# ghostop14/gr-clenabled

Measured on AMD Instinct MI355X. Metric: MSamples/sec (complex-float) through clFFT 4096 fwd + window + shift, higher is better.
Workload: dtype f32; 1 GPU; BASELINE configs[1]: forward clFFT 4096-pt complex, blackman window + fftshift, 16384 frames/step/GPU device-resident (1 GiB in+out); fft_size=4096, parallelism=replica-per-gpu x1

## Files before the change

gr-clenabled_amd/csrc/fft.hip:

```cpp
#include <cmath>
#include <cstdlib>
#include <vector>

#include "common.h"
#include "fft_core.hpp"
#include "fft_mr.h"

using namespace fftc;
#ifndef MI355_FFT_WPE
#define MI355_FFT_WPE 3
#endif

namespace {

typedef float f2v __attribute__((ext_vector_type(2)));

template <int N, bool REAL, class G>
__device__ __forceinline__ void load_group(c32 (&v)[16], const void *__restrict__ in, int grp, int tid, int nframes, int in_xor)
{
    using P = Plan<N>;
    constexpr int TH = G::TH, PTS = G::PTS, F = G::F, R0 = P::radix(0), B0 = N / R0;
    const int frames_left = nframes - grp * F;
    if constexpr (N <= 64) {
        (void)in_xor;
#pragma unroll
        for (int k = 0; k < 16; k++) {
            const unsigned e = (unsigned)(tid + TH * k);
            const bool ok = (int)(e / N) < frames_left;
            if constexpr (REAL) {
                const float x = __builtin_nontemporal_load((const float *)in + (size_t)grp * PTS + (ok ? e : 0u));
                v[k] = mk(ok ? x : 0.f, 0.f);
            } else {
                const f2v x = __builtin_nontemporal_load((const f2v *)in + (size_t)grp * PTS + (ok ? e : 0u));
                v[k] = ok ? mk(x.x, x.y) : mk(0.f, 0.f);
            }
        }
        return;
    }
#pragma unroll
    for (int q = 0; q < 16 / R0; q++) {
        const int g = tid + TH * q, fr = g / B0;
        const bool ok = (F == 1) || fr < frames_left;
        const unsigned off = (unsigned)((ok ? fr * N : 0) + (g % B0));
#pragma unroll
        for (int r = 0; r < R0; r++) {
            const unsigned e = off + (unsigned)((r * B0) ^ in_xor);
            if constexpr (REAL) {
                const float x = __builtin_nontemporal_load((const float *)in + (size_t)grp * PTS + e);
                v[q * R0 + r] = mk(ok ? x : 0.f, 0.f);
            } else {
                const f2v x = __builtin_nontemporal_load((const f2v *)in + (size_t)grp * PTS + e);
                v[q * R0 + r] = ok ? mk(x.x, x.y) : mk(0.f, 0.f);
            }
        }
    }
}

template <int N, int SIGN, bool REAL, int PF, class G>
__global__ __launch_bounds__(G::TH, (N <= 4096 ? (PF == 2 ? 2 : MI355_FFT_WPE) : 1)) void k_fft(const void *__restrict__ in, c32 *__restrict__ out,
                                                                 const float *__restrict__ window,
                                                                 const c32 *__restrict__ twtab, int nframes, int ngroups,
                                                                 int shift)
{
    using P = Plan<N>;
    constexpr int TH = G::TH, PTS = G::PTS, F = G::F, NP = P::NP;
    constexpr bool SMALL = N <= 64;
    constexpr int PAD = (N / P::radix(0)) > 1 ? (N / P::radix(0)) : 1;
    constexpr int LDS_SLOTS = SMALL ? PTS + (PTS / N) * PAD : (NP > 1 ? PTS : 1);
    __shared__ c32 lds[LDS_SLOTS];
    const int tid0 = threadIdx.x;
    const int in_xor = (SIGN > 0 && shift) ? (N >> 1) : 0;
    const int out_xor = (SIGN < 0 && shift) ? (N >> 1) : 0;

    TwRegs<N> tw;
    load_twiddles<N, false, G>(tw, tid0, twtab);
    constexpr int R0 = P::radix(0), B0 = N / R0;
    float win[16];
    if constexpr (SMALL) {
        win[0] = window[tid0 % N];
    } else {
#pragma unroll
        for (int q = 0; q < 16 / R0; q++) {
            const int j = (tid0 + TH * q) % B0;
#pragma unroll
            for (int r = 0; r < R0; r++) win[q * R0 + r] = window[j + ((r * B0) ^ in_xor)];
        }
    }

    auto body = [&](c32 (&cur)[16], int grp, int tid) {
        const int frames_left = nframes - grp * F;
        c32 v[16];
        if constexpr (SMALL) {
            const float wv = win[0];
            const int pos = (tid % N) ^ in_xor, fr0 = tid / N;
#pragma unroll
            for (int k = 0; k < 16; k++) {
                const int fr = fr0 + k * (TH / N);
                lds[fr * (N + PAD) + pos] = scale(cur[k], wv);
            }
            __syncthreads();
#pragma unroll
            for (int q = 0; q < 16 / R0; q++) {
                const int g = tid + TH * q, base = (g / B0) * (N + PAD) + (g % B0);
#pragma unroll
                for (int r = 0; r < R0; r++) v[q * R0 + r] = lds[base + r * B0];
            }
            __syncthreads();
        } else {
#pragma unroll
            for (int s = 0; s < 16; s++) v[s] = scale(cur[s], win[s]);
        }
        transform_regs<N, SIGN, false, G>(v, tw, lds, tid);
        if constexpr (SMALL) {
            constexpr int RL = P::radix(NP - 1), BL = N / RL;
            if constexpr (NP > 1) __syncthreads();
#pragma unroll
            for (int q = 0; q < 16 / RL; q++) {
                const int g = tid + TH * q, base = (g / BL) * (N + PAD) + (g % BL);
#pragma unroll
                for (int s = 0; s < RL; s++) lds[base + ((orev<RL>(s) * BL) ^ out_xor)] = v[q * RL + s];
            }
            __syncthreads();
            f2v *__restrict__ out_g = (f2v *)out + (size_t)grp * PTS;
            const int pos = tid % N, fr0 = tid / N;
#pragma unroll
            for (int k = 0; k < 16; k++) {
                const int fr = fr0 + k * (TH / N);
                if (fr < frames_left) {
                    const c32 z = lds[fr * (N + PAD) + pos];
                    f2v o;
                    o.x = z.x;
                    o.y = z.y;
                    __builtin_nontemporal_store(o, out_g + tid + TH * k);
                }
            }
        } else {
            constexpr int RL = P::radix(NP - 1), BL = N / RL;
            f2v *__restrict__ out_g = (f2v *)out + (size_t)grp * PTS;
#pragma unroll
            for (int q = 0; q < 16 / RL; q++) {
                const int g = tid + TH * q, fr = g / BL;
                const unsigned off = (unsigned)(fr * N + (g % BL));
                if ((F == 1) || fr < frames_left) {
#pragma unroll
                    for (int s = 0; s < RL; s++) {
                        f2v o;
                        o.x = v[q * RL + s].x;
                        o.y = v[q * RL + s].y;
                        __builtin_nontemporal_store(o, out_g + off + (unsigned)((orev<RL>(s) * BL) ^ out_xor));
                    }
                }
            }
        }
        if constexpr (NP > 1 || SMALL) __syncthreads();
    };
    const int stride = gridDim.x;
    if constexpr (PF == 2) {
        c32 b0[16], b1[16], b2[16];
        int grp = blockIdx.x;
        if (grp < ngroups) load_group<N, REAL, G>(b0, in, grp, tid0, nframes, in_xor);
        if (grp + stride < ngroups) load_group<N, REAL, G>(b1, in, grp + stride, tid0, nframes, in_xor);
#define MI355_FFT_STEP(CUR, FREE)                                                                   \
        {                                                                                           \
            if (grp >= ngroups) break;                                                              \
            int tid = tid0;                                                                         \
            asm volatile("" : "+v"(tid));                                                           \
            if (grp + 2 * stride < ngroups) load_group<N, REAL, G>(FREE, in, grp + 2 * stride, tid, nframes, in_xor); \
            __builtin_amdgcn_sched_barrier(0);                                                      \
            body(CUR, grp, tid);                                                                    \
            grp += stride;                                                                          \
        }
        for (;;) {
            MI355_FFT_STEP(b0, b2)
            MI355_FFT_STEP(b1, b0)
            MI355_FFT_STEP(b2, b1)
        }
#undef MI355_FFT_STEP
    } else {
        c32 cur[16];
        if ((int)blockIdx.x < ngroups) load_group<N, REAL, G>(cur, in, blockIdx.x, tid0, nframes, in_xor);
        for (int grp = blockIdx.x; grp < ngroups; grp += stride) {
            int tid = tid0;
            asm volatile("" : "+v"(tid));
            c32 nxt[16];
            if constexpr (PF == 1) {
                const int gnext = grp + stride;
                if (gnext < ngroups) load_group<N, REAL, G>(nxt, in, gnext, tid, nframes, in_xor);
                __builtin_amdgcn_sched_barrier(0);
            } else if (grp != (int)blockIdx.x) {
                load_group<N, REAL, G>(cur, in, grp, tid, nframes, in_xor);
            }
            body(cur, grp, tid);
            if constexpr (PF == 1) {
#pragma unroll
                for (int s = 0; s < 16; s++) cur[s] = nxt[s];
            }
        }
    }
}

typedef float f4v __attribute__((ext_vector_type(4)));
__host__ __device__ constexpr float cos128(int m)
{
    constexpr float t[128] = {1.0f, 0.99879545f, 0.99518472f, 0.989176512f, 0.980785251f, 0.970031261f, 0.956940353f, 0.941544056f, 0.923879504f, 0.903989315f, 0.881921291f, 0.857728601f, 0.831469595f, 0.803207517f, 0.773010433f, 0.740951121f, 0.707106769f, 0.671558976f, 0.634393275f, 0.59569931f, 0.555570245f, 0.514102757f, 0.471396744f, 0.427555084f, 0.382683426f, 0.336889863f, 0.290284663f, 0.242980182f, 0.195090324f, 0.146730468f, 0.0980171412f, 0.0490676761f, 0.0f, -0.0490676761f, -0.0980171412f, -0.146730468f, -0.195090324f, -0.242980182f, -0.290284663f, -0.336889863f, -0.382683426f, -0.427555084f, -0.471396744f, -0.514102757f, -0.555570245f, -0.59569931f, -0.634393275f, -0.671558976f, -0.707106769f, -0.740951121f, -0.773010433f, -0.803207517f, -0.831469595f, -0.857728601f, -0.881921291f, -0.903989315f, -0.923879504f, -0.941544056f, -0.956940353f, -0.970031261f, -0.980785251f, -0.989176512f, -0.99518472f, -0.99879545f, -1.0f, -0.99879545f, -0.99518472f, -0.989176512f, -0.980785251f, -0.970031261f, -0.956940353f, -0.941544056f, -0.923879504f, -0.903989315f, -0.881921291f, -0.857728601f, -0.831469595f, -0.803207517f, -0.773010433f, -0.740951121f, -0.707106769f, -0.671558976f, -0.634393275f, -0.59569931f, -0.555570245f, -0.514102757f, -0.471396744f, -0.427555084f, -0.382683426f, -0.336889863f, -0.290284663f, -0.242980182f, -0.195090324f, -0.146730468f, -0.0980171412f, -0.0490676761f, 0.0f, 0.0490676761f, 0.0980171412f, 0.146730468f, 0.195090324f, 0.242980182f, 0.290284663f, 0.336889863f, 0.382683426f, 0.427555084f, 0.471396744f, 0.514102757f, 0.555570245f, 0.59569931f, 0.634393275f, 0.671558976f, 0.707106769f, 0.740951121f, 0.773010433f, 0.803207517f, 0.831469595f, 0.857728601f, 0.881921291f, 0.903989315f, 0.923879504f, 0.941544056f, 0.956940353f, 0.970031261f, 0.980785251f, 0.989176512f, 0.99518472f, 0.99879545f};
    return t[m & 127];
}
__host__ __device__ constexpr float circ_cos(int m, int circ) { return cos128(m * (128 / circ)); }
__host__ __device__ constexpr float circ_sin(int m, int circ) { return cos128(m * (128 / circ) - 32); }
static_assert(circ_cos(0, 128) == 1.0f && circ_cos(32, 128) == 0.0f && circ_cos(16, 128) == 0.707106781f && circ_sin(32, 128) == 1.0f &&
                  circ_sin(8, 64) == 0.707106781f && circ_cos(16, 32) == -1.0f, "twiddle table");

template <int SIGN, bool REAL>
__global__ __launch_bounds__(512, 2) void k_fft_32k(const void *__restrict__ in, c32 *__restrict__ out, const float *__restrict__ window,
                                                    const c32 *__restrict__ twN, int nframes, int shift)
{
    constexpr int N = 32768, NS = 4096, S = 8, H = 4, BL = 256;
    using G = Geo<NS>;
    __shared__ c32 sm[4 * NS];
    const int set = threadIdx.x >> 8, tid0 = threadIdx.x & 255;
    c32 *lds = sm + set * 2 * NS;
    const int in_xor = (SIGN > 0 && shift) ? 8 : 0;
    const int m_xor = (SIGN < 0 && shift) ? (S / 2) : 0;

#ifndef PFR32K
#define PFR32K 0
#endif
    constexpr int PFW = REAL ? 2 : 4, PFR = REAL ? 2 * PFR32K : PFR32K;
    f4v pf[PFR > 0 ? PFR : 1][PFW];
    auto fetch = [&](int frame, int j, int tid, f4v (&t)[PFW]) {
        const unsigned n = (unsigned)(tid + (((8 * set + j) ^ in_xor) * BL));
        const f4v *p = (const f4v *)in + (size_t)frame * (REAL ? N / 4 : N / 2) + (size_t)n * PFW;
#pragma unroll
        for (int k = 0; k < PFW; k++) t[k] = p[k];
    };
    if ((int)blockIdx.x < nframes) {
#pragma unroll
        for (int j = 0; j < PFR; j++) fetch(blockIdx.x, j, tid0, pf[j]);
    }
    for (int frame = blockIdx.x; frame < nframes; frame += gridDim.x) {
        int tid = tid0;
        asm volatile("" : "+v"(tid));
        c32 v[H][16];
        auto load_frame = [&](auto set_tag) {
            constexpr int SET = decltype(set_tag)::value, OTHER = 1 - SET;
#pragma unroll
            for (int j = 0; j < 8; j++) {
                const int r = 8 * SET + j;
                const unsigned n = (unsigned)(tid + ((r ^ in_xor) * BL));
// ... 510 lines not shown
#pragma unroll
            for (int h = 0; h < 2; h++) {
                const int n2 = c0 + fr + 8 * h;
                const c32 base = twN[(int)(((long long)n2 * j) & nmask)], g1 = twN[(int)(((long long)n2 * BL) & nmask)];
                const c32 g2 = cmul(g1, g1), g4 = cmul(g2, g2), g8 = cmul(g4, g4);
                c32 gp[16];
                gp[0] = base;
                gp[1] = cmul(base, g1);
                gp[2] = cmul(base, g2);
                gp[3] = cmul(gp[2], g1);
                gp[4] = cmul(base, g4);
                gp[5] = cmul(gp[4], g1);
                gp[6] = cmul(gp[4], g2);
                gp[7] = cmul(gp[6], g1);
#pragma unroll
                for (int m = 0; m < 8; m++) gp[8 + m] = cmul(gp[m], g8);
                f2v *__restrict__ o = (f2v *)out + (size_t)frame * frame_elems + (size_t)n2 * NR + j;
#pragma unroll
                for (int t = 0; t < 16; t++) {
                    const c32 z = cmul(h ? vb[t] : va[t], gp[orev<16>(t)]);
                    f2v zz;
                    zz.x = z.x;
                    zz.y = z.y;
                    o[orev<16>(t) * BL] = zz;
                }
            }
            __syncthreads();
        } else {
            __syncthreads();
#pragma unroll
            for (int q = 0; q < 16 / RL; q++) {
                const int g = tid + TH * q, fr = g / BL, j = g % BL;
#pragma unroll
                for (int t = 0; t < RL; t++) {
                    tile_lds[fr * CS + j + orev<RL>(t) * BL] = va[q * RL + t];
                    tile_lds[(fr + 8) * CS + j + orev<RL>(t) * BL] = vb[q * RL + t];
                }
            }
            __syncthreads();
#pragma unroll
            for (int i = 0; i < 32; i++) {
                const int e = tid + TH * i, col = e & 15, row = e >> 4;
                const c32 z = tile_lds[col * CS + row];
                f2v zz;
                zz.x = z.x;
                zz.y = z.y;
                __builtin_nontemporal_store(zz, (f2v *)out + (size_t)frame * frame_elems + (size_t)(row ^ row_xor) * ld + c0 + col);
            }
            __syncthreads();
        }
    }
}

template <int N, class G>
int launch_g(mi355_ctx *ctx, int sign, const void *in, void *out, const float *window, const void *tw, int nframes, int shift,
             int real_in, hipStream_t st)
{
    constexpr int F = G::F, TH = G::TH, WAVES = TH / 64;
    int ngroups = (nframes + F - 1) / F;
    int cus = ctx->num_cus > 0 ? ctx->num_cus : 256;
    int pf = getenv("MI355_FFT_PREFETCH") ? atoi(getenv("MI355_FFT_PREFETCH")) : -1;
    const bool persistent2 = N <= 4096 && WAVES == 4 && ngroups >= cus * 2 * 8;
    if (pf < 0) pf = persistent2 ? 1 : 0;
    int grid = (N <= 4096) ? mi355_balanced_grid(ctx, ngroups, 32 / WAVES, 64 / WAVES, 0.015) : mi355_balanced_grid(ctx, ngroups, 1, 1);
    if (pf == 1 && persistent2) grid = cus * 2;
    if (const char *e = getenv("MI355_FFT_WG_PER_CU")) {
        if (atoi(e) > 0) grid = ngroups < cus * atoi(e) ? ngroups : cus * atoi(e);
    }
#define LAUNCH_FFT(SG, RL)                                                                                              \
    do {                                                                                                                     \
        if (pf == 2)                                                                                                         \
            hipLaunchKernelGGL((k_fft<N, SG, RL, 2, G>), dim3(grid), dim3(TH), 0, st, in, (c32 *)out, window, (const c32 *)tw, \
                               nframes, ngroups, shift);                                                                     \
        else if (pf == 1)                                                                                                    \
            hipLaunchKernelGGL((k_fft<N, SG, RL, 1, G>), dim3(grid), dim3(TH), 0, st, in, (c32 *)out, window, (const c32 *)tw, \
                               nframes, ngroups, shift);                                                                     \
        else                                                                                                                 \
            hipLaunchKernelGGL((k_fft<N, SG, RL, 0, G>), dim3(grid), dim3(TH), 0, st, in, (c32 *)out, window,                \
                               (const c32 *)tw, nframes, ngroups, shift);                                                    \
    } while (0)
    if (sign < 0) { if (real_in) LAUNCH_FFT(-1, true); else LAUNCH_FFT(-1, false); }
    else          { if (real_in) LAUNCH_FFT(1, true);  else LAUNCH_FFT(1, false); }
#undef LAUNCH_FFT
    MI355_HIP(hipGetLastError());
    return MI355_OK;
}

template <int N>
int launch_n(mi355_ctx *ctx, int sign, const void *in, void *out, const float *window, const void *tw, int nframes, int shift,
             int real_in, hipStream_t st)
{
    if constexpr (N >= 16 && N <= 1024) {
        static const bool wave = getenv("MI355_FFT_WAVE_GEO") ? atoi(getenv("MI355_FFT_WAVE_GEO")) != 0 : false;
        if (wave) return launch_g<N, GeoW<N>>(ctx, sign, in, out, window, tw, nframes, shift, real_in, st);
    }
    if constexpr (N == 32768) return launch_s<N>(ctx, sign, in, out, window, tw, nframes, shift, real_in, st);
    else if constexpr (N == 8192 || N == 16384) {
        static const bool whole = getenv("MI355_FFT_WHOLE_FRAME") ? atoi(getenv("MI355_FFT_WHOLE_FRAME")) != 0 : false;
        if (!whole) return launch_s<N>(ctx, sign, in, out, window, tw, nframes, shift, real_in, st);
    }
    if constexpr (N != 32768) return launch_g<N, Geo<N>>(ctx, sign, in, out, window, tw, nframes, shift, real_in, st);
}

int launch_fft(mi355_ctx *ctx, int n, int sign, const void *in, void *out, const float *window, const void *tw, int nframes,
               int shift, int real_in, hipStream_t st)
{
    switch (n) {
#define CASE_N(NN) case NN: return launch_n<NN>(ctx, sign, in, out, window, tw, nframes, shift, real_in, st)
        CASE_N(2); CASE_N(4); CASE_N(8); CASE_N(16); CASE_N(32); CASE_N(64); CASE_N(128); CASE_N(256); CASE_N(512);
        CASE_N(1024); CASE_N(2048); CASE_N(4096); CASE_N(8192); CASE_N(16384); CASE_N(32768);
#undef CASE_N
    }
    mi355_set_error("fft size %d unsupported (power of two, 2..32768)", n);
    return MI355_ERR_UNSUPPORTED;
}

}

struct mi355_fft {
    mi355_ctx *ctx;
    int n, sign, dtype, nstreams, shift;
    float *d_window;
    void *d_tw;
    HostPipe pipe;
    MrPlan mr;
    MrTilePlan mrt;
    int m = 0;
    void *d_pre = nullptr, *d_post = nullptr, *d_bspec = nullptr;
    void *d_twm_f = nullptr, *d_twm_i = nullptr;
    float *d_ones = nullptr;
    mi355_fft *sub_f = nullptr, *sub_i = nullptr;
    void *d_wa = nullptr, *d_wb = nullptr;
    size_t cap_frames = 0;
    bool two_kernel = false;
    int tile_n1 = 0, tile_n2 = 0;
    std::mutex ws_lock;
    hipEvent_t ws_done = nullptr;
    bool ws_used = false;
};

namespace {

__global__ __launch_bounds__(256) void k_blu_pre(const void *__restrict__ in, c32 *__restrict__ A, const c32 *__restrict__ pre,
                                                 const int *__restrict__ src, int N, int M, long long total, int real_in)
{
    for (long long e = (long long)blockIdx.x * 256 + threadIdx.x; e < total; e += (long long)gridDim.x * 256) {
        const long long f = e / M;
        const int m = (int)(e - f * M);
        c32 v = mk(0.f, 0.f);
        if (m < N) {
            const int i = src[m];
            const c32 x = real_in ? mk(((const float *)in)[f * N + i], 0.f) : ((const c32 *)in)[f * N + i];
            v = cmul(x, pre[m]);
        }
        A[e] = v;
    }
}

__global__ __launch_bounds__(256) void k_blu_mul(c32 *__restrict__ B, const c32 *__restrict__ bspec, int M, long long total)
{
    for (long long e = (long long)blockIdx.x * 256 + threadIdx.x; e < total; e += (long long)gridDim.x * 256)
        B[e] = cmul(B[e], bspec[e & (M - 1)]);
}

__global__ __launch_bounds__(256) void k_blu_post(const c32 *__restrict__ A, c32 *__restrict__ out, const c32 *__restrict__ post,
                                                  int N, int M, long long total, int lo)
{
    for (long long e = (long long)blockIdx.x * 256 + threadIdx.x; e < total; e += (long long)gridDim.x * 256) {
        const long long f = e / N;
        const int p = (int)(e - f * N);
        const int k = lo ? (p < N - lo ? p + lo : p - (N - lo)) : p;
        out[e] = cmul(A[f * M + k], post[k]);
    }
}

template <int M, bool REAL>
__global__ __launch_bounds__(Geo<M>::TH, Geo<M>::WPE) void k_chirpz(const void *__restrict__ in, c32 *__restrict__ out,
                                                                   const c32 *__restrict__ pre, const int *__restrict__ src,
                                                                   const c32 *__restrict__ post, const c32 *__restrict__ bspec,
                                                                   const c32 *__restrict__ tw_fwd, const c32 *__restrict__ tw_inv,
                                                                   int N, int nframes, int ngroups, int lo)
{
    using G = Geo<M>;
    using PF = Plan<M, false>;
    using PI = Plan<M, true>;
    constexpr int TH = G::TH, F = G::F, NP = PF::NP;
    constexpr int RL = PF::radix(NP - 1), BL = M / RL;
    static_assert(PI::radix(0) == RL, "inverse plan must start with the forward plan's last radix");
    extern __shared__ __attribute__((aligned(16))) c32 chirp_lds[];
    c32 *lds = chirp_lds;
    const int tid0 = threadIdx.x;
// ... 308 lines not shown
                const long long total = (long long)nf * 65536;
                long long blocks = (total + 255) / 256;
                if (blocks > (long long)cus * 16) blocks = (long long)cus * 16;
                const int mx = (h->sign < 0 && h->shift) ? S2 / 2 : 0;
#define COMB2F(SS) do { if (h->sign < 0) COMB2(SS, -1, 1, (const c32 *)h->d_wb, dst, (const c32 *)h->d_tw, total, 65536, (long long)N, 65536LL, 0LL, 0LL, 1, N - 1, mx); \
                        else             COMB2(SS, 1, 1, (const c32 *)h->d_wb, dst, (const c32 *)h->d_tw, total, 65536, (long long)N, 65536LL, 0LL, 0LL, 1, N - 1, mx); } while (0)
                if (S2 == 2) COMB2F(2); else if (S2 == 4) COMB2F(4); else if (S2 == 8) COMB2F(8); else COMB2F(16);
#undef COMB2F
            }
            MI355_HIP(hipGetLastError());
            continue;
        }
#undef COMB2
        const long long total = (long long)nf * 4096;
        long long blocks = (total + 255) / 256;
        if (blocks > (long long)cus * 16) blocks = (long long)cus * 16;
#define COMB(SS, SG) hipLaunchKernelGGL((k_fft_combine<SS, SG>), dim3((unsigned)blocks), dim3(256), 0, st, (const c32 *)h->d_wa, dst, (const c32 *)h->d_tw, total, m_xor)
        if (S == 8) { if (h->sign < 0) COMB(8, -1); else COMB(8, 1); }
        else        { if (h->sign < 0) COMB(16, -1); else COMB(16, 1); }
#undef COMB
        MI355_HIP(hipGetLastError());
    }
    return ws_release(h, st);
}

int launch_mr_tile(mi355_fft *h, const void *in, void *out, int nframes, hipStream_t st)
{
    const size_t N = (size_t)h->n;
    size_t chunk = ((size_t)256 << 20) / (N * 8);
    if (chunk < 1) chunk = 1;
    if (chunk > (size_t)nframes) chunk = (size_t)nframes;
    std::lock_guard<std::mutex> ws_guard(h->ws_lock);
    {
        const int rc = ws_acquire(h, st, chunk > h->cap_frames);
        if (rc) return rc;
    }
    if (chunk > h->cap_frames) {
        MI355_HIP(hipStreamSynchronize(st));
        if (h->d_wa) (void)hipFree(h->d_wa);
        h->d_wa = nullptr; h->cap_frames = 0;
        MI355_HIP(hipMalloc(&h->d_wa, chunk * N * 8));
        h->cap_frames = chunk;
    }
    const size_t isz = h->dtype == MI355_DTYPE_FLOAT ? 4 : 8;
    for (size_t f0 = 0; f0 < (size_t)nframes; f0 += chunk) {
        const int nf = (int)((size_t)nframes - f0 < chunk ? (size_t)nframes - f0 : chunk);
        const int rc = mi355_fft_mr_tile_launch(h->mrt, h->ctx, h->sign, (const char *)in + f0 * N * isz, h->d_wa, (char *)out + f0 * N * 8, h->d_window, nf,
                                                h->shift, h->dtype == MI355_DTYPE_FLOAT, st);
        if (rc) return rc;
    }
    return ws_release(h, st);
}

int launch_handle(mi355_fft *h, const void *in, void *out, int nvec, hipStream_t st)
{
    if (h->mrt.n) return launch_mr_tile(h, in, out, nvec, st);
    if (h->mr.n) return mi355_fft_mr_launch(h->mr, h->ctx, h->sign, in, out, h->d_window, nvec, h->shift, h->dtype == MI355_DTYPE_FLOAT, st);
    if (h->m) return launch_bluestein(h, in, out, nvec, st);
    if (h->n > 32768 || (h->n == 32768 && h->two_kernel)) return launch_big(h, in, out, nvec, st);
    return launch_fft(h->ctx, h->n, h->sign, in, out, h->d_window, h->d_tw, nvec, h->shift, h->dtype == MI355_DTYPE_FLOAT, st);
}

void host_fft_pow2(std::vector<double> &re, std::vector<double> &im, int sign)
{
    const int n = (int)re.size();
    for (int i = 1, j = 0; i < n; i++) {
        int bit = n >> 1;
        for (; j & bit; bit >>= 1) j ^= bit;
        j ^= bit;
        if (i < j) { std::swap(re[i], re[j]); std::swap(im[i], im[j]); }
    }
    std::vector<double> cr(n / 2 > 0 ? n / 2 : 1), ci(n / 2 > 0 ? n / 2 : 1);
    for (int k = 0; k < n / 2; k++) {
        const double a = sign * 2.0 * M_PI * (double)k / (double)n;
        cr[k] = cos(a);
        ci[k] = sin(a);
    }
    for (int len = 2; len <= n; len <<= 1) {
        const int step = n / len;
        for (int i = 0; i < n; i += len)
            for (int k = 0; k < len / 2; k++) {
                const double wr = cr[(size_t)k * step], wi = ci[(size_t)k * step];
                const int p = i + k, q = p + len / 2;
                const double tr = re[q] * wr - im[q] * wi, ti = re[q] * wi + im[q] * wr;
                re[q] = re[p] - tr; im[q] = im[p] - ti;
                re[p] += tr; im[p] += ti;
            }
    }
}

int upload(mi355_ctx *ctx, void **d, const void *src, size_t bytes)
{
    if (hipMalloc(d, bytes) != hipSuccess) return MI355_ERR_NOMEM;
    if (mi355_upload(ctx, *d, src, bytes) != hipSuccess) return MI355_ERR_HIP;
    return MI355_OK;
}

std::vector<float> twiddle_table(int n, int sign)
{
    std::vector<float> tw;
    tw.reserve(2 * (size_t)n + 8192);
    for (int k = 0; k < n; k++) {
        const double a = sign * 2.0 * M_PI * (double)k / (double)n;
        tw.push_back((float)cos(a));
        tw.push_back((float)sin(a));
    }
    if (n > 4096)
        for (int k = 0; k < 4096; k++) {
            const double a = sign * 2.0 * M_PI * (double)k / 4096.0;
            tw.push_back((float)cos(a));
            tw.push_back((float)sin(a));
        }
    return tw;
// ... 68 lines not shown
    if (!h) return MI355_ERR_NOMEM;
    h->ctx = ctx; h->n = fft_size;
    h->sign = (direction == MI355_FFT_FORWARD) ? -1 : 1;
    h->dtype = dtype; h->nstreams = num_streams; h->shift = shift ? 1 : 0;
    h->d_window = nullptr; h->d_tw = nullptr;
    auto fail = [&](int rc) { mi355_fft_destroy(h); return rc; };
    if (hipSetDevice(ctx->device) != hipSuccess) return fail(MI355_ERR_HIP);
    std::vector<float> tw(2 * (size_t)fft_size);
    for (int k = 0; k < fft_size; k++) {
        double a = h->sign * 2.0 * M_PI * (double)k / (double)fft_size;
        tw[2 * k] = (float)cos(a);
        tw[2 * k + 1] = (float)sin(a);
    }
    if (fft_size > 4096) {
        for (int k = 0; k < 4096; k++) {
            double a = h->sign * 2.0 * M_PI * (double)k / 4096.0;
            tw.push_back((float)cos(a));
            tw.push_back((float)sin(a));
        }
    }
    if (pow2 && fft_size >= 65536 && fft_size <= 1048576 && !getenv("MI355_FFT_NO_TILE")) {
        int lg = 0;
        while ((1 << lg) < fft_size) lg++;
        h->tile_n1 = lg == 17 ? 256 : 1 << ((lg + 1) / 2);
        if (const char *e = getenv("MI355_FFT_TILE_N1")) {
            const int v = atoi(e);
            if ((v == 256 || v == 512 || v == 1024) && fft_size / v >= 256 && fft_size / v <= 1024) h->tile_n1 = v;
        }
        h->tile_n2 = fft_size / h->tile_n1;
        for (int nr : {h->tile_n1, h->tile_n2})
            for (int k = 0; k < nr; k++) {
                double a = h->sign * 2.0 * M_PI * (double)k / (double)nr;
                tw.push_back((float)cos(a));
                tw.push_back((float)sin(a));
            }
    }
    if (hipMalloc(&h->d_tw, tw.size() * sizeof(float)) != hipSuccess) return fail(MI355_ERR_NOMEM);
    if (mi355_upload(ctx, h->d_tw, tw.data(), tw.size() * sizeof(float)) != hipSuccess) return fail(MI355_ERR_HIP);
    {
        std::vector<float> w(fft_size, 1.0f);
        if (window_len) memcpy(w.data(), window, sizeof(float) * (size_t)fft_size);
        h->two_kernel = pow2 && (fft_size > 32768 || (fft_size == 32768 && getenv("MI355_FFT_32768_TWO_KERNELS") != nullptr));
        if (h->two_kernel && !h->tile_n1) {
            const int S = fft_size / 4096;
            std::vector<float> p((size_t)fft_size);
            for (int sq = 0; sq < S / 4; sq++)
                for (int n = 0; n < 4096; n++)
                    for (int j = 0; j < 4; j++) p[((size_t)sq * 4096 + n) * 4 + j] = w[(size_t)n * S + 4 * sq + j];
            w.swap(p);
        }
        if (hipMalloc((void **)&h->d_window, sizeof(float) * (size_t)fft_size) != hipSuccess) return fail(MI355_ERR_NOMEM);
        if (mi355_upload(ctx, h->d_window, w.data(), sizeof(float) * (size_t)fft_size) != hipSuccess)
            return fail(MI355_ERR_HIP);
    }
    int rc = h->pipe.init(ctx);
    if (rc) return fail(rc);
    if (!pow2) {
        std::vector<float> mtw;
        if (!getenv("MI355_FFT_NO_MR") && mi355_fft_mr_plan(fft_size, h->sign, 0, &h->mr, &mtw)) {
            auto put = [&](MrPlan &pl, const std::vector<float> &t) {
                if (hipMalloc(&pl.d_tw, t.size() * sizeof(float)) != hipSuccess) return (int)MI355_ERR_NOMEM;
                return mi355_upload(ctx, pl.d_tw, t.data(), t.size() * sizeof(float)) != hipSuccess ? (int)MI355_ERR_HIP : (int)MI355_OK;
            };
            int known = mi355_fft_mr_cached_variant(fft_size);
            if (known < 0 && !getenv("MI355_FFT_MR_TIMED_VARIANT")) known = (fft_size == 96 || fft_size == 100 || fft_size == 2400) ? 1 : 0;
            if (const char *e = getenv("MI355_FFT_MR_VARIANT")) known = atoi(e) != 0 ? 1 : 0;
            MrPlan alt;
            std::vector<float> atw;
            const bool have_alt = mi355_fft_mr_plan(fft_size, h->sign, 1, &alt, &atw) && (alt.npass != h->mr.npass || alt.per_thread != h->mr.per_thread);
            if (known == 1 && have_alt) {
                h->mr = alt;
                mtw.swap(atw);
            }
            if ((rc = put(h->mr, mtw))) return fail(rc);
            float ms0 = -1.f, ms1 = -1.f;
            if ((rc = mi355_fft_mr_tune(&h->mr, ctx, h->sign, h->d_window, &ms0))) return fail(rc);
            if (known < 0 && have_alt && ms0 > 0.f && getenv("MI355_FFT_MR_TIMED_VARIANT")) {
                if ((rc = put(alt, atw))) { if (alt.d_tw) (void)hipFree(alt.d_tw); return fail(rc); }
                rc = mi355_fft_mr_tune(&alt, ctx, h->sign, h->d_window, &ms1);
                if (rc) { (void)hipFree(alt.d_tw); return fail(rc); }
                if (ms1 > 0.f && ms1 < ms0 * 0.90f) {
                    (void)hipFree(h->mr.d_tw);
                    h->mr = alt;
                } else {
                    (void)hipFree(alt.d_tw);
                }
            }
            if (ms0 > 0.f) {
                mi355_fft_mr_remember(h->mr);
                mi355_log(ctx, MI355_LOG_INFO, "clFFT %d points (mixed radix): %d passes, %d threads x %d frame(s) per workgroup measured fastest", fft_size,
                          h->mr.npass, h->mr.threads, h->mr.frames);
            }
        } else {
            h->mr.n = 0;
            std::vector<float> twa, twb;
            if (!getenv("MI355_FFT_NO_MR") && mi355_fft_mr_tile_plan(fft_size, h->sign, &h->mrt, &twa, &twb)) {
                h->mrt.a.d_tw = h->mrt.b.d_tw = nullptr;
                if (hipMalloc(&h->mrt.a.d_tw, twa.size() * sizeof(float) + 8) != hipSuccess) return fail(MI355_ERR_NOMEM);
                if (hipMalloc(&h->mrt.b.d_tw, twb.size() * sizeof(float) + 8) != hipSuccess) return fail(MI355_ERR_NOMEM);
                if (!twa.empty() && mi355_upload(ctx, h->mrt.a.d_tw, twa.data(), twa.size() * sizeof(float)) != hipSuccess) return fail(MI355_ERR_HIP);
                if (!twb.empty() && mi355_upload(ctx, h->mrt.b.d_tw, twb.data(), twb.size() * sizeof(float)) != hipSuccess) return fail(MI355_ERR_HIP);
                h->mrt.d_twn = h->d_tw;
            } else {
                h->mrt.n = 0;
                rc = setup_bluestein(h, window_len ? window : nullptr);
                if (rc) return fail(rc);
// ... 12 lines not shown
{
    MI355_REQUIRE(buf && buf_len > 0, "NULL argument");
    const bool pow2 = fft_size >= 2 && (fft_size & (fft_size - 1)) == 0;
    if (fft_size < 2 || (pow2 && fft_size > 16777216) || (!pow2 && fft_size > 8388608)) {
        snprintf(buf, (size_t)buf_len, "unsupported (powers of two 2..16777216, any other size 3..8388608)");
        return MI355_ERR_UNSUPPORTED;
    }
    if (pow2) {
        if (fft_size <= 32768) snprintf(buf, (size_t)buf_len, "one pass");
        else if (fft_size <= 1048576) {
            int lg = 0;
            while ((1 << lg) < fft_size) lg++;
            const int n1 = lg == 17 ? 256 : 1 << ((lg + 1) / 2);
            snprintf(buf, (size_t)buf_len, "two tile passes %d x %d", n1, fft_size / n1);
        } else snprintf(buf, (size_t)buf_len, "four passes");
        return MI355_OK;
    }
    MrPlan mp;
    std::vector<float> tw;
    if (mi355_fft_mr_plan(fft_size, -1, 0, &mp, &tw)) {
        int at = snprintf(buf, (size_t)buf_len, "mixed radix ");
        for (int p = 0; p < mp.npass && at < buf_len; p++) at += snprintf(buf + at, (size_t)(buf_len - at), p ? " x %d" : "%d", mp.pass[p].radix);
        return MI355_OK;
    }
    MrTilePlan tp;
    std::vector<float> twb;
    if (mi355_fft_mr_tile_plan(fft_size, -1, &tp, &tw, &twb)) {
        snprintf(buf, (size_t)buf_len, "mixed radix, two passes %d x %d", tp.n1, tp.n2);
        return MI355_OK;
    }
    int m = 256;
    while (m < 2 * fft_size - 1) m <<= 1;
    snprintf(buf, (size_t)buf_len, "chirp-z, m = %d%s", m, m <= 16384 ? " (fused)" : "");
    return MI355_OK;
}

const MrPlan *mi355_fft_mr_plan_of(const mi355_fft *h, int *sign)
{
    if (!h || !h->mr.n) return nullptr;
    if (sign) *sign = h->sign;
    return &h->mr;
}

extern "C" int mi355_fft_destroy(mi355_fft *h)
{
    if (!h) return MI355_OK;
    (void)hipSetDevice(h->ctx->device);
    h->pipe.release();
    if (h->d_window) (void)hipFree(h->d_window);
    if (h->d_tw) (void)hipFree(h->d_tw);
    if (h->mr.d_tw) (void)hipFree(h->mr.d_tw);
    if (h->mrt.a.d_tw) (void)hipFree(h->mrt.a.d_tw);
    if (h->mrt.b.d_tw) (void)hipFree(h->mrt.b.d_tw);
    for (void *p : {h->d_pre, h->d_post, h->d_bspec, h->d_twm_f, h->d_twm_i, (void *)h->d_ones, h->d_wa, h->d_wb})
        if (p) (void)hipFree(p);
    if (h->ws_done) (void)hipEventDestroy(h->ws_done);
    if (h->sub_f) (void)mi355_fft_destroy(h->sub_f);
    if (h->sub_i) (void)mi355_fft_destroy(h->sub_i);
    delete h;
    return MI355_OK;
}

extern "C" int mi355_fft_work_dev(mi355_fft *h, int nvec, const void *in, void *out, void *stream)
{
    MI355_REQUIRE(h != nullptr, "handle is NULL");
    if (nvec <= 0) return MI355_OK;
    MI355_REQUIRE(in && out, "NULL buffer");
    MI355_REQUIRE((reinterpret_cast<uintptr_t>(in) & 7u) == 0 && (reinterpret_cast<uintptr_t>(out) & 7u) == 0,
                  "device buffers must be 8-byte aligned");
    MI355_REQUIRE(h->m != 0 || h->n <= 4096 || (reinterpret_cast<uintptr_t>(in) & 15u) == 0,
                  "device input of an 8192/16384-point transform must be 16-byte aligned");
    MI355_HIP(hipSetDevice(h->ctx->device));
    return launch_handle(h, in, out, nvec, mi355_pick_stream(h->ctx, stream));
}

extern "C" int mi355_fft_work(mi355_fft *h, int nvec, const void *const *in_streams, void *const *out_streams)
{
    MI355_REQUIRE(h != nullptr, "handle is NULL");
    if (nvec <= 0) return MI355_OK;
    MI355_REQUIRE(in_streams && out_streams, "NULL stream arrays");
    std::lock_guard<std::mutex> g(h->ctx->lock);
    MI355_HIP(hipSetDevice(h->ctx->device));
    const size_t isz = mi355_dtype_size(h->dtype), in_frame = isz * (size_t)h->n, out_frame = 8 * (size_t)h->n;
    size_t chunk_frames = mi355_chunk_bytes((size_t)nvec * out_frame) / out_frame;
    if (chunk_frames < 1) chunk_frames = 1;
    size_t first = (size_t)nvec < chunk_frames ? (size_t)nvec : chunk_frames;
    size_t inb = first * in_frame;
    const int nslots = first * out_frame >= ((size_t)32 << 20) ? 2 : HostPipe::kSlots;
    int rc = h->pipe.ensure(1, &inb, first * out_frame, nslots);
    if (rc) return rc;
    HostPipe &p = h->pipe;
    if ((size_t)nvec <= chunk_frames && mi355_direct_ok((size_t)nvec * out_frame)) {
        hipStream_t st = h->ctx->stream[0];
        for (int s_i = 0; s_i < h->nstreams; s_i++) {
            MI355_REQUIRE(in_streams[s_i] && out_streams[s_i], "NULL stream buffer");
            mi355_copy(p.h_in[0][0], in_streams[s_i], (size_t)nvec * in_frame);
            rc = launch_handle(h, p.h_in[0][0], p.h_out[0], nvec, st);
            if (rc) return rc;
            MI355_HIP(mi355_direct_sync(st));
            mi355_copy(out_streams[s_i], p.h_out[0], (size_t)nvec * out_frame);
        }
        return MI355_OK;
    }
    size_t nchunks = ((size_t)nvec + chunk_frames - 1) / chunk_frames;
    char *pend_dst[HostPipe::kSlots] = {};
    size_t pend_bytes[HostPipe::kSlots] = {};
    size_t seq = 0;
// ... 33 lines not shown
```

Baseline: 372,900 MSamples/s.

## Add atomic work-claiming dynamic schedule for persistent 4096-point FFT kernel

```diff
diff --git a/gr-clenabled_amd/csrc/fft.hip b/gr-clenabled_amd/csrc/fft.hip
--- a/gr-clenabled_amd/csrc/fft.hip
+++ b/gr-clenabled_amd/csrc/fft.hip
@@ -56,11 +56,27 @@
     }
 }
 
-template <int N, int SIGN, bool REAL, int PF, class G>
+constexpr int kClaimWords = 8;
+constexpr int kClaimStride = 64;
+constexpr int kClaimStatic = 3;
+constexpr int kClaimSetWords = kClaimWords * kClaimStride;
+constexpr int kClaimSets = 8;
+constexpr int kTsSlots = 64;
+
+__device__ __forceinline__ unsigned hw_cu_id()
+{
+    const unsigned hw = __builtin_amdgcn_s_getreg((3 << 11) | (8 << 6) | 4);
+    const unsigned se = __builtin_amdgcn_s_getreg((1 << 11) | (13 << 6) | 4);
+    const unsigned xcc = __builtin_amdgcn_s_getreg((3 << 11) | (0 << 6) | 20);
+    return (xcc << 16) | (se << 8) | hw;
+}
+
+template <int N, int SIGN, bool REAL, int PF, class G, bool DYN = false, bool TS = false>
 __global__ __launch_bounds__(G::TH, (N <= 4096 ? (PF == 2 ? 2 : MI355_FFT_WPE) : 1)) void k_fft(const void *__restrict__ in, c32 *__restrict__ out,
                                                                  const float *__restrict__ window,
                                                                  const c32 *__restrict__ twtab, int nframes, int ngroups,
-                                                                 int shift)
+                                                                 int shift, unsigned *__restrict__ claims,
+                                                                 unsigned long long *__restrict__ ts)
 {
     using P = Plan<N>;
     constexpr int TH = G::TH, PTS = G::PTS, F = G::F, NP = P::NP;
@@ -155,6 +171,13 @@
         if constexpr (NP > 1 || SMALL) __syncthreads();
     };
     const int stride = gridDim.x;
+    static_assert(!TS || PF == 1, "stamps: the persistent schedule only");
+    if constexpr (TS) {
+        if (tid0 == 0) {
+            ts[(size_t)blockIdx.x * kTsSlots + 0] = (unsigned long long)wall_clock64();
+            ts[(size_t)blockIdx.x * kTsSlots + 3] = hw_cu_id();
+        }
+    }
     if constexpr (PF == 2) {
         c32 b0[16], b1[16], b2[16];
         int grp = blockIdx.x;
@@ -176,8 +199,59 @@
             MI355_FFT_STEP(b2, b1)
         }
 #undef MI355_FFT_STEP
+    } else if constexpr (PF == 1 && DYN) {
+        static_assert(NP > 1 || SMALL, "the transform ends with a workgroup barrier");
+        __shared__ int claimed[2];
+        const int nb = (int)gridDim.x >> 3, b = (int)blockIdx.x >> 3, cls = b % kClaimWords;
+        const int m = (nb / kClaimWords + (cls < nb % kClaimWords ? 1 : 0)) * 8 + (nb % kClaimWords == cls ? ((int)gridDim.x & 7) : 0);
+        const int rank = (b / kClaimWords) * 8 + ((int)blockIdx.x & 7);
+        const int lo = (int)((long long)cls * ngroups / kClaimWords), hi = (int)((long long)(cls + 1) * ngroups / kClaimWords);
+        const unsigned nclaim = (unsigned)(hi - lo - kClaimStatic * m);
+        const unsigned last = (unsigned)(hi - lo - (kClaimStatic - 2) * m - 1);
+        unsigned *word = claims + cls * kClaimStride;
+        unsigned t_prev = ~0u;
+        bool claiming = true;
+        int g = lo + rank, g_next = g + m;
+        [[maybe_unused]] int done = 0;
+        c32 cur[16];
+        load_group<N, REAL, G>(cur, in, g, tid0, nframes, in_xor);
+        for (int k = 0; k < ngroups; k++) {
+            int tid = tid0;
+            asm volatile("" : "+v"(tid));
+            unsigned t_new = ~0u;
+            if (tid0 == 0 && claiming) t_new = atomicAdd(word, 1u);
+            __builtin_amdgcn_sched_barrier(0);
+            c32 nxt[16];
+            if (g_next >= 0) load_group<N, REAL, G>(nxt, in, g_next, tid, nframes, in_xor);
+            __builtin_amdgcn_sched_barrier(0);
+            if (tid0 == 0 && k > 0) {
+                const bool ok = t_prev < nclaim;
+                claimed[k & 1] = ok ? lo + kClaimStatic * m + (int)t_prev : -1;
+                if (!ok) claiming = false;
+                if (t_prev == last) atomicExch(word, 0u);
+            }
+            t_prev = t_new;
+            body(cur, g, tid);
+            if constexpr (TS) {
+                done++;
+                if (tid0 == 0 && (done & 7) == 0 && (done >> 3) <= kTsSlots - 8)
+                    ts[(size_t)blockIdx.x * kTsSlots + 7 + (done >> 3)] = (unsigned long long)wall_clock64();
+            }
+            if (g_next < 0) break;
+            g = g_next;
+            g_next = k == 0 ? lo + rank + 2 * m : claimed[k & 1];
+#pragma unroll
+            for (int s = 0; s < 16; s++) cur[s] = nxt[s];
+        }
+        if constexpr (TS) {
+            if (tid0 == 0) {
+                ts[(size_t)blockIdx.x * kTsSlots + 1] = (unsigned long long)wall_clock64();
+                ts[(size_t)blockIdx.x * kTsSlots + 2] = (unsigned long long)done;
+            }
+        }
     } else {
         c32 cur[16];
+        [[maybe_unused]] int done = 0;
         if ((int)blockIdx.x < ngroups) load_group<N, REAL, G>(cur, in, blockIdx.x, tid0, nframes, in_xor);
         for (int grp = blockIdx.x; grp < ngroups; grp += stride) {
             int tid = tid0;
@@ -191,9 +265,20 @@
                 load_group<N, REAL, G>(cur, in, grp, tid, nframes, in_xor);
             }
             body(cur, grp, tid);
+            if constexpr (TS) {
+                done++;
+                if (tid0 == 0 && (done & 7) == 0 && (done >> 3) <= kTsSlots - 8)
+                    ts[(size_t)blockIdx.x * kTsSlots + 7 + (done >> 3)] = (unsigned long long)wall_clock64();
+            }
             if constexpr (PF == 1) {
 #pragma unroll
                 for (int s = 0; s < 16; s++) cur[s] = nxt[s];
+            }
+        }
+        if constexpr (TS) {
+            if (tid0 == 0) {
+                ts[(size_t)blockIdx.x * kTsSlots + 1] = (unsigned long long)wall_clock64();
+                ts[(size_t)blockIdx.x * kTsSlots + 2] = (unsigned long long)done;
             }
         }
     }
@@ -810,9 +895,52 @@
     }
 }
 
+unsigned long long *stamps_buffer(int grid)
+{
+    static std::mutex mu;
+    static unsigned long long *d = nullptr;
+    static int cap = 0;
+    std::lock_guard<std::mutex> g(mu);
+    if (cap < grid) {
+        if (d) (void)hipFree(d);
+        d = nullptr;
+        cap = 0;
+        if (hipMalloc(&d, (size_t)grid * kTsSlots * 8) != hipSuccess) return nullptr;
+        cap = grid;
+    }
+    return d;
+}
+
+int dump_stamps(const unsigned long long *d_ts, int n, int sign, int sched, int grid, int ngroups, hipStream_t st)
+{
+    MI355_HIP(hipStreamSynchronize(st));
+    std::vector<unsigned long long> h((size_t)grid * kTsSlots);
+    MI355_HIP(hipMemcpy(h.data(), d_ts, h.size() * 8, hipMemcpyDeviceToHost));
+    unsigned long long t0 = ~0ull, t1 = 0;
+    for (int b = 0; b < grid; b++) {
+        t0 = std::min(t0, h[(size_t)b * kTsSlots]);
+        t1 = std::max(t1, h[(size_t)b * kTsSlots + 1]);
+    }
+    fprintf(stderr, "[fft stamps] N %d sign %d sched %d: %d workgroups, %d groups, first start to last end %.2f us\n", n, sign, sched, grid,
+            ngroups, (double)(t1 - t0) * 0.01);
+    if (const char *path = getenv("MI355_FFT_TS_FILE")) {
+        if (FILE *f = fopen(path, "a")) {
+            fprintf(f, "# n %d sign %d sched %d grid %d ngroups %d\n", n, sign, sched, grid, ngroups);
+            for (int b = 0; b < grid; b++) {
+                const unsigned long long *r = &h[(size_t)b * kTsSlots];
+                fprintf(f, "%d %llu %llu %llu %llu", b, r[3], r[0], r[1], r[2]);
+                for (int i = 8; i < kTsSlots && r[i]; i++) fprintf(f, " %llu", r[i]);
+                fprintf(f, "\n");
+            }
+            fclose(f);
+        }
+    }
+    return MI355_OK;
+}
+
 template <int N, class G>
 int launch_g(mi355_ctx *ctx, int sign, const void *in, void *out, const float *window, const void *tw, int nframes, int shift,
-             int real_in, hipStream_t st)
+             int real_in, hipStream_t st, unsigned *claims)
 {
     constexpr int F = G::F, TH = G::TH, WAVES = TH / 64;
     int ngroups = (nframes + F - 1) / F;
@@ -825,46 +953,57 @@
     if (const char *e = getenv("MI355_FFT_WG_PER_CU")) {
         if (atoi(e) > 0) grid = ngroups < cus * atoi(e) ? ngroups : cus * atoi(e);
     }
-#define LAUNCH_FFT(SG, RL)                                                                                              \
-    do {                                                                                                                     \
-        if (pf == 2)                                                                                                         \
-            hipLaunchKernelGGL((k_fft<N, SG, RL, 2, G>), dim3(grid), dim3(TH), 0, st, in, (c32 *)out, window, (const c32 *)tw, \
-                               nframes, ngroups, shift);                                                                     \
-        else if (pf == 1)                                                                                                    \
-            hipLaunchKernelGGL((k_fft<N, SG, RL, 1, G>), dim3(grid), dim3(TH), 0, st, in, (c32 *)out, window, (const c32 *)tw, \
-                               nframes, ngroups, shift);                                                                     \
-        else                                                                                                                 \
-            hipLaunchKernelGGL((k_fft<N, SG, RL, 0, G>), dim3(grid), dim3(TH), 0, st, in, (c32 *)out, window,                \
-                               (const c32 *)tw, nframes, ngroups, shift);                                                    \
+    int sched = getenv("MI355_FFT_SCHED") ? atoi(getenv("MI355_FFT_SCHED")) : (N == 4096 ? 1 : 0);
+    if (!(pf == 1 && persistent2 && claims && grid >= 8 * kClaimWords &&
+          ngroups / kClaimWords >= kClaimStatic * ((grid + 8 * kClaimWords - 1) / (8 * kClaimWords)) * 8))
+        sched = 0;
+    if (sched != 1) claims = nullptr;
+    unsigned long long *ts = nullptr;
+    if (pf == 1 && getenv("MI355_FFT_TS")) {
+        ts = stamps_buffer(grid);
+        if (ts) MI355_HIP(hipMemsetAsync(ts, 0, (size_t)grid * kTsSlots * 8, st));
+    }
+#define LAUNCH_FFT_K(...) hipLaunchKernelGGL((k_fft<__VA_ARGS__>), dim3(grid), dim3(TH), 0, st, in, (c32 *)out, window, (const c32 *)tw, \
+                                                nframes, ngroups, shift, claims, ts)
+#define LAUNCH_FFT(SG, RL)                                                                      \
+    do {                                                                                             \
+        if (pf == 2) LAUNCH_FFT_K(N, SG, RL, 2, G);                                                  \
+        else if (pf == 1 && sched == 1 && ts) LAUNCH_FFT_K(N, SG, RL, 1, G, true, true);             \
+        else if (pf == 1 && sched == 1) LAUNCH_FFT_K(N, SG, RL, 1, G, true);                         \
+        else if (pf == 1 && ts) LAUNCH_FFT_K(N, SG, RL, 1, G, false, true);                          \
+        else if (pf == 1) LAUNCH_FFT_K(N, SG, RL, 1, G);                                             \
+        else LAUNCH_FFT_K(N, SG, RL, 0, G);                                                          \
     } while (0)
     if (sign < 0) { if (real_in) LAUNCH_FFT(-1, true); else LAUNCH_FFT(-1, false); }
     else          { if (real_in) LAUNCH_FFT(1, true);  else LAUNCH_FFT(1, false); }
 #undef LAUNCH_FFT
+#undef LAUNCH_FFT_K
     MI355_HIP(hipGetLastError());
+    if (ts) return dump_stamps(ts, N, sign, sched, grid, ngroups, st);
     return MI355_OK;
 }
 
 template <int N>
 int launch_n(mi355_ctx *ctx, int sign, const void *in, void *out, const float *window, const void *tw, int nframes, int shift,
-             int real_in, hipStream_t st)
+             int real_in, hipStream_t st, unsigned *claims)
 {
     if constexpr (N >= 16 && N <= 1024) {
         static const bool wave = getenv("MI355_FFT_WAVE_GEO") ? atoi(getenv("MI355_FFT_WAVE_GEO")) != 0 : false;
-        if (wave) return launch_g<N, GeoW<N>>(ctx, sign, in, out, window, tw, nframes, shift, real_in, st);
+        if (wave) return launch_g<N, GeoW<N>>(ctx, sign, in, out, window, tw, nframes, shift, real_in, st, claims);
     }
     if constexpr (N == 32768) return launch_s<N>(ctx, sign, in, out, window, tw, nframes, shift, real_in, st);
     else if constexpr (N == 8192 || N == 16384) {
         static const bool whole = getenv("MI355_FFT_WHOLE_FRAME") ? atoi(getenv("MI355_FFT_WHOLE_FRAME")) != 0 : false;
         if (!whole) return launch_s<N>(ctx, sign, in, out, window, tw, nframes, shift, real_in, st);
     }
-    if constexpr (N != 32768) return launch_g<N, Geo<N>>(ctx, sign, in, out, window, tw, nframes, shift, real_in, st);
+    if constexpr (N != 32768) return launch_g<N, Geo<N>>(ctx, sign, in, out, window, tw, nframes, shift, real_in, st, claims);
 }
 
 int launch_fft(mi355_ctx *ctx, int n, int sign, const void *in, void *out, const float *window, const void *tw, int nframes,
-               int shift, int real_in, hipStream_t st)
+               int shift, int real_in, hipStream_t st, unsigned *claims = nullptr)
 {
     switch (n) {
-#define CASE_N(NN) case NN: return launch_n<NN>(ctx, sign, in, out, window, tw, nframes, shift, real_in, st)
+#define CASE_N(NN) case NN: return launch_n<NN>(ctx, sign, in, out, window, tw, nframes, shift, real_in, st, claims)
         CASE_N(2); CASE_N(4); CASE_N(8); CASE_N(16); CASE_N(32); CASE_N(64); CASE_N(128); CASE_N(256); CASE_N(512);
         CASE_N(1024); CASE_N(2048); CASE_N(4096); CASE_N(8192); CASE_N(16384); CASE_N(32768);
 #undef CASE_N
@@ -895,6 +1034,10 @@
     std::mutex ws_lock;
     hipEvent_t ws_done = nullptr;
     bool ws_used = false;
+    unsigned *d_claims = nullptr;
+    hipStream_t claim_st[kClaimSets] = {};
+    int nclaim_st = 0;
+    std::mutex claim_lock;
 };
 
 namespace {
@@ -1309,13 +1452,31 @@
     return ws_release(h, st);
 }
 
+unsigned *claim_words(mi355_fft *h, hipStream_t st)
+{
+    if (!h->d_claims || st == hipStreamPerThread) return nullptr;
+    hipStreamCaptureStatus cs = hipStreamCaptureStatusNone;
+    if (hipStreamIsCapturing(st, &cs) != hipSuccess) {
+        (void)hipGetLastError();
+        return nullptr;
+    }
+    if (cs != hipStreamCaptureStatusNone) return nullptr;
+    std::lock_guard<std::mutex> g(h->claim_lock);
+    for (int i = 0; i < h->nclaim_st; i++)
+        if (h->claim_st[i] == st) return h->d_claims + (size_t)i * kClaimSetWords;
+    if (h->nclaim_st == kClaimSets) return nullptr;
+    h->claim_st[h->nclaim_st] = st;
+    return h->d_claims + (size_t)h->nclaim_st++ * kClaimSetWords;
+}
+
 int launch_handle(mi355_fft *h, const void *in, void *out, int nvec, hipStream_t st)
 {
     if (h->mrt.n) return launch_mr_tile(h, in, out, nvec, st);
     if (h->mr.n) return mi355_fft_mr_launch(h->mr, h->ctx, h->sign, in, out, h->d_window, nvec, h->shift, h->dtype == MI355_DTYPE_FLOAT, st);
     if (h->m) return launch_bluestein(h, in, out, nvec, st);
     if (h->n > 32768 || (h->n == 32768 && h->two_kernel)) return launch_big(h, in, out, nvec, st);
-    return launch_fft(h->ctx, h->n, h->sign, in, out, h->d_window, h->d_tw, nvec, h->shift, h->dtype == MI355_DTYPE_FLOAT, st);
+    return launch_fft(h->ctx, h->n, h->sign, in, out, h->d_window, h->d_tw, nvec, h->shift, h->dtype == MI355_DTYPE_FLOAT, st,
+                      claim_words(h, st));
 }
 
 void host_fft_pow2(std::vector<double> &re, std::vector<double> &im, int sign)
@@ -1490,6 +1651,11 @@
         if (hipMalloc((void **)&h->d_window, sizeof(float) * (size_t)fft_size) != hipSuccess) return fail(MI355_ERR_NOMEM);
         if (mi355_upload(ctx, h->d_window, w.data(), sizeof(float) * (size_t)fft_size) != hipSuccess)
             return fail(MI355_ERR_HIP);
+    }
+    if (pow2 && fft_size <= 4096) {
+        const std::vector<unsigned> zero((size_t)kClaimSets * kClaimSetWords, 0u);
+        if (hipMalloc(&h->d_claims, zero.size() * sizeof(unsigned)) != hipSuccess) return fail(MI355_ERR_NOMEM);
+        if (mi355_upload(ctx, h->d_claims, zero.data(), zero.size() * sizeof(unsigned)) != hipSuccess) return fail(MI355_ERR_HIP);
     }
     int rc = h->pipe.init(ctx);
     if (rc) return fail(rc);
@@ -1608,7 +1774,7 @@
     if (h->mr.d_tw) (void)hipFree(h->mr.d_tw);
     if (h->mrt.a.d_tw) (void)hipFree(h->mrt.a.d_tw);
     if (h->mrt.b.d_tw) (void)hipFree(h->mrt.b.d_tw);
-    for (void *p : {h->d_pre, h->d_post, h->d_bspec, h->d_twm_f, h->d_twm_i, (void *)h->d_ones, h->d_wa, h->d_wb})
+    for (void *p : {h->d_pre, h->d_post, h->d_bspec, h->d_twm_f, h->d_twm_i, (void *)h->d_ones, h->d_wa, h->d_wb, (void *)h->d_claims})
         if (p) (void)hipFree(p);
     if (h->ws_done) (void)hipEventDestroy(h->ws_done);
     if (h->sub_f) (void)mi355_fft_destroy(h->sub_f);
```

Result: faster. 389,500 MSamples/s (median of 6 runs) (+4.4%).
